# simonmeister/UnFlow

Hardware: AMD Instinct MI355X
Metric: image-pairs/s (fwd+bwd) FlowNetC 384x512 (higher is better)
Workload: dtype f32; 1 GPU; FlowNetC unsupervised step: bidirectional fwd + census/2nd-order loss pyramid + bwd + L2/Adam, 4 pairs/GPU, 384x512, 441-ch correlation (BASELINE configs[1]); global_batch=4, height=384, width=512, parallelism=dp1, hipgraph=True

## Files before the change

unflow_amd/csrc/conv_igemm.hip:

```cpp
#include "igemm_shared.h"
#include "options.h"

namespace {
using namespace igemm;

constexpr int LDK = BK + 4;

struct GatherParams : GatherGeom {
  const float* src;
  const float* w;
  const float* bias;
  float* dst;
  float* partial;
  const float* act_src;
  int lds, ldd, ld_act, act_lo, act_hi;
  int nsplit;
  int leaky, accumulate;
  unsigned cs_magic;
  PlaneOut pl;
};

__device__ __forceinline__ float4 ldg4(const float* p) { return *reinterpret_cast<const float4*>(p); }

typedef __bf16 bf16x8 __attribute__((ext_vector_type(8)));
constexpr bool kEarlyLoads = true;
constexpr int LDH = BK;
__device__ __forceinline__ int swz_off(int row, int kquad) {
  return row * LDH + 8 * ((kquad >> 1) ^ ((row >> 2) & 3)) + 4 * (kquad & 1);
}
__device__ __forceinline__ void split_store(unsigned short* __restrict__ dst, int plane_stride, const float4 v) {
  const unsigned h0 = cvt_pk_bf16(v.x, v.y), h1 = cvt_pk_bf16(v.z, v.w);
  const float r0 = v.x - __uint_as_float(h0 << 16), r1 = v.y - __uint_as_float(h0 & 0xffff0000u);
  const float r2 = v.z - __uint_as_float(h1 << 16), r3 = v.w - __uint_as_float(h1 & 0xffff0000u);
  const unsigned m0 = cvt_pk_bf16(r0, r1), m1 = cvt_pk_bf16(r2, r3);
  const float s0 = r0 - __uint_as_float(m0 << 16), s1 = r1 - __uint_as_float(m0 & 0xffff0000u);
  const float s2 = r2 - __uint_as_float(m1 << 16), s3 = r3 - __uint_as_float(m1 & 0xffff0000u);
  *reinterpret_cast<uint2*>(dst) = make_uint2(h0, h1);
  *reinterpret_cast<uint2*>(dst + plane_stride) = make_uint2(m0, m1);
  *reinterpret_cast<uint2*>(dst + 2 * plane_stride) = make_uint2(cvt_pk_bf16(s0, s1), cvt_pk_bf16(s2, s3));
}

template <int BM, int BN, int WM, int WN, bool B_NK, int MATH = 0>
__global__ __launch_bounds__(256) void igemm_gather_kernel(const GatherParams p) {
  constexpr int TM = WM / 32, TN = WN / 32;
  constexpr int WAVES_N = BN / WN;
  static_assert((BM / WM) * WAVES_N == 4, "4 waves");
  constexpr int A_ELEMS = BM * LDK;
  constexpr int A_PLANE = BM * LDH, B_PLANE = BN * LDH;
  constexpr int AR = BM / 32;
  constexpr int BR_NK = BN / 32;
  constexpr int KG = 256 / BN;
  constexpr int BQ_KN = 8 / KG;
  constexpr int NB = B_NK ? BR_NK : BQ_KN;

  extern __shared__ __attribute__((aligned(16))) float smem[];
  float* As = smem;
  float* Bs = smem + A_ELEMS;
  unsigned short* Ah = reinterpret_cast<unsigned short*>(smem);
  unsigned short* Bh = Ah + 3 * A_PLANE;
  int* pix = MATH ? reinterpret_cast<int*>(Bh + 3 * B_PLANE) : reinterpret_cast<int*>(smem + A_ELEMS + BN * LDK);

  const int tid = threadIdx.x, lane = tid & 63, wid = tid >> 6;
  const int wm = wid / WAVES_N, wn = wid % WAVES_N;
  const int cls_id = blockIdx.z % p.ncls, split = blockIdx.z / p.ncls;
  const TapClass tc = p.cls[cls_id];
  const int M = p.B * p.Hg * p.Wg;
  const int m0 = blockIdx.x * BM, n0 = blockIdx.y * BN;
  const int ntaps = tc.nty * tc.ntx;
  const int Cq = p.Cs >> 2;
  const int Ktot = ntaps * p.Cs;
  const int KT = (Ktot + BK - 1) / BK;
  const int kt_per = (KT + p.nsplit - 1) / p.nsplit;
  const int kt0 = split * kt_per;
  const int kt1 = min(KT, kt0 + kt_per);

  const __amdgpu_buffer_rsrc_t src_rs =
      make_rsrc(p.src, ((size_t)p.B * p.Hs * p.Ws - 1) * (size_t)p.lds * 4 + (size_t)p.Cs * 4);
  const __amdgpu_buffer_rsrc_t w_rs = make_rsrc(p.w, (size_t)p.wtaps * p.Cs * p.N * 4);

  const int kq = tid & 7;
  int a_y[AR], a_x[AR], a_lin[AR];
#pragma unroll
  for (int i = 0; i < AR; i++) {
    const int m = m0 + (tid >> 3) + 32 * i;
    if (m < M) {
      const int xg = m % p.Wg, t = m / p.Wg;
      const int yg = t % p.Hg, b = t / p.Hg;
      a_y[i] = yg * p.sm;
      a_x[i] = xg * p.sm;
      a_lin[i] = b * p.Hs * p.Ws + a_y[i] * p.Ws + a_x[i];
    } else {
      a_y[i] = -(1 << 28);
      a_x[i] = 0;
      a_lin[i] = 0;
    }
  }
  if (tid < BM) {
    const int m = m0 + tid;
    int v = -1;
    if (m < M) {
      const int xg = m % p.Wg, t = m / p.Wg;
      const int yg = t % p.Hg, b = t / p.Hg;
      v = (b * p.Hd + yg * p.so + tc.py) * p.Wd + xg * p.so + tc.px;
    }
    pix[tid] = v;
  }
  int b_row[NB];
  int kn_voff = 0;
  int kn_kg = 0;
  if constexpr (B_NK) {
#pragma unroll
    for (int i = 0; i < NB; i++) {
      const int n = n0 + (tid >> 3) + 32 * i;
      b_row[i] = n < p.N ? n * p.Cs * 4 : OOB_MARK;
    }
  } else {
    const int n = n0 + (tid % BN);
    kn_voff = n < p.N ? n * 4 : OOB_MARK;
    kn_kg = __builtin_amdgcn_readfirstlane(tid / BN);
  }
  const int lds4 = p.lds * 4;

  const int adv_t = 8 / Cq, adv_c = 8 - adv_t * Cq;
  const unsigned ntx_magic = (65536u + (unsigned)tc.ntx - 1u) / (unsigned)tc.ntx;
  int q_tap, q_c4;
  {
    const unsigned q = (unsigned)kt0 * 8u + (unsigned)kq;
    q_tap = (int)(q / (unsigned)Cq);
    q_c4 = (int)(q - (unsigned)q_tap * (unsigned)Cq);
  }
  bool live = kt0 < kt1;

  float4 ra[AR];
  float4 rb[NB];
  int dy, dx, a_tile, w_tile;

  auto piece_begin = [&]() {
    const int ty = (int)(((unsigned)q_tap * ntx_magic) >> 16), tx = q_tap - ty * tc.ntx;
    const bool kvalid = live && q_tap < ntaps;
    dy = tc.dy0 + ty * p.dstep;
    dx = tc.dx0 + tx * p.dstep;
    const int cofs = q_c4 * 16;
    a_tile = kvalid ? (dy * p.Ws + dx) * lds4 + cofs : OOB_MARK;
    if constexpr (B_NK) {
      const int widx = (tc.ky0 + ty * p.kstep) * p.KW + tc.kx0 + tx * p.kstep;
      w_tile = kvalid ? widx * p.N * p.Cs * 4 + cofs : OOB_MARK;
    }
  };
  auto piece_a = [&](int i, float4* RA) {
    const int y = a_y[i] + dy, x = a_x[i] + dx;
    const bool inb = (unsigned)y < (unsigned)p.Hs && (unsigned)x < (unsigned)p.Ws;
    const int voff = inb ? a_lin[i] * lds4 + a_tile : OOB_MARK;
    RA[i] = buf_ld4(src_rs, voff, 0);
  };
  auto piece_b = [&](int i, int kt_next, float4* RB) {
    if constexpr (B_NK) {
      RB[i] = buf_ld4(w_rs, b_row[i] + w_tile, 0);
    } else {
      const int kk = kt_next * BK + 4 * (kn_kg + KG * i);
      float v[4];
#pragma unroll
      for (int j = 0; j < 4; j++) v[j] = buf_ld1(w_rs, kn_voff, min(kk + j, Ktot - 1) * p.N * 4);
      RB[i] = make_float4(v[0], v[1], v[2], v[3]);
    }
  };
  auto piece_end = [&]() {
    q_c4 += adv_c;
    q_tap += adv_t;
    const bool wrap = q_c4 >= Cq;
    q_c4 -= wrap ? Cq : 0;
    q_tap += wrap ? 1 : 0;
  };
  auto piece_set = [&](int step, int kt_next, float4* RA, float4* RB) {
    if (step == 0) piece_begin();
    if (step >= 1 && step <= AR) piece_a(step - 1, RA);
    if (step > AR && step <= AR + NB) piece_b(step - AR - 1, kt_next, RB);
    if (step == AR + NB + 1) piece_end();
  };
  auto piece = [&](int step, int kt_next) { piece_set(step, kt_next, ra, rb); };
  static_assert(AR + NB + 2 <= 16, "pieces must fit the 16 steps");

  auto store_set = [&](const float4* RA, const float4* RB) {
#pragma unroll
    for (int i = 0; i < AR; i++) split_store(Ah + swz_off((tid >> 3) + 32 * i, kq), A_PLANE, RA[i]);
    if constexpr (B_NK) {
#pragma unroll
      for (int i = 0; i < BR_NK; i++) split_store(Bh + swz_off((tid >> 3) + 32 * i, kq), B_PLANE, RB[i]);
    } else {
#pragma unroll
      for (int i = 0; i < BQ_KN; i++) split_store(Bh + swz_off(tid % BN, (tid / BN) + KG * i), B_PLANE, RB[i]);
    }
  };
  auto store_tile = [&]() {
    if constexpr (MATH == 1) {
      store_set(ra, rb);
      return;
    }
#pragma unroll
    for (int i = 0; i < AR; i++)
      *reinterpret_cast<float4*>(As + ((tid >> 3) + 32 * i) * LDK + kq * 4) = ra[i];
    if constexpr (B_NK) {
#pragma unroll
      for (int i = 0; i < BR_NK; i++)
        *reinterpret_cast<float4*>(Bs + ((tid >> 3) + 32 * i) * LDK + kq * 4) = rb[i];
    } else {
#pragma unroll
      for (int i = 0; i < BQ_KN; i++)
        *reinterpret_cast<float4*>(Bs + (tid % BN) * LDK + 4 * ((tid / BN) + KG * i)) = rb[i];
    }
  };

  f32x16 acc[TM][TN];
#pragma unroll
  for (int i = 0; i < TM; i++)
#pragma unroll
    for (int j = 0; j < TN; j++)
#pragma unroll
      for (int r = 0; r < 16; r++) acc[i][j][r] = 0.f;

  const int l31 = lane & 31, lh = lane >> 5;
#pragma unroll
  for (int st = 0; st < 16; st++) piece(st, kt0);
  store_tile();
  __syncthreads();
  const float* a_rd = As + (wm * WM + l31) * LDK + 16 * lh;
  const float* b_rd = Bs + (wn * WN + l31) * LDK + 16 * lh;
  const unsigned short* ah_rd = Ah + (wm * WM + l31) * LDH;
  const unsigned short* bh_rd = Bh + (wn * WN + l31) * LDH;
  const int gsw = lh ^ ((l31 >> 2) & 3);
  constexpr bool EARLY_LOADS = kEarlyLoads;
  auto mfma_phase = [&](int kload, float4* RA, float4* RB) {
#pragma unroll
    for (int slab = 0; slab < 2; slab++) {
      bf16x8 av[3][TM], bv[3][TN];
#pragma unroll
      for (int pl = 0; pl < 3; pl++) {
#pragma unroll
        for (int i = 0; i < TM; i++)
          av[pl][i] = *reinterpret_cast<const bf16x8*>(ah_rd + pl * A_PLANE + i * 32 * LDH + 8 * (gsw ^ (2 * slab)));
#pragma unroll
        for (int j = 0; j < TN; j++)
          bv[pl][j] = *reinterpret_cast<const bf16x8*>(bh_rd + pl * B_PLANE + j * 32 * LDH + 8 * (gsw ^ (2 * slab)));
      }
      constexpr int ta[6] = {2, 0, 1, 1, 0, 0}, tb[6] = {0, 2, 1, 0, 1, 0};
#pragma unroll
      for (int t = 0; t < 6; t++) {
#pragma unroll
        for (int i = 0; i < TM; i++)
#pragma unroll
          for (int j = 0; j < TN; j++)
            acc[i][j] = __builtin_amdgcn_mfma_f32_32x32x16_bf16(av[ta[t]][i], bv[tb[t]][j], acc[i][j], 0, 0, 0);
        if (EARLY_LOADS) {
          piece_set(2 * (slab * 6 + t), kload, RA, RB);
          piece_set(2 * (slab * 6 + t) + 1, kload, RA, RB);
        } else {
          piece_set(slab * 6 + t, kload, RA, RB);
        }
        __builtin_amdgcn_sched_barrier(0);
      }
    }
    if (!EARLY_LOADS) {
#pragma unroll
      for (int st = 12; st < 16; st++) piece_set(st, kload, RA, RB);
    }
  };
  for (int kt = kt0; kt < kt1; kt++) {
    live = kt + 1 < kt1;
    if constexpr (MATH == 1) {
      mfma_phase(kt + 1, ra, rb);
    } else {
#pragma unroll
    for (int j4 = 0; j4 < 4; j4++) {
      float4 av[TM], bv[TN];
#pragma unroll
      for (int i = 0; i < TM; i++) av[i] = *reinterpret_cast<const float4*>(a_rd + i * 32 * LDK + 4 * j4);
#pragma unroll
      for (int j = 0; j < TN; j++) bv[j] = *reinterpret_cast<const float4*>(b_rd + j * 32 * LDK + 4 * j4);
#pragma unroll
      for (int e = 0; e < 4; e++) {
#pragma unroll
        for (int i = 0; i < TM; i++)
#pragma unroll
          for (int j = 0; j < TN; j++)
            acc[i][j] = __builtin_amdgcn_mfma_f32_32x32x2f32((&av[i].x)[e], (&bv[j].x)[e], acc[i][j], 0, 0, 0);
        piece(j4 * 4 + e, kt + 1);
        __builtin_amdgcn_sched_barrier(0);
      }
    }
    }
    __syncthreads();
    store_tile();
    __syncthreads();
  }

  const bool to_partial = p.nsplit > 1;
#pragma unroll
  for (int i = 0; i < TM; i++)
#pragma unroll
    for (int r = 0; r < 16; r++) {
      const int row = wm * WM + i * 32 + (r & 3) + 8 * (r >> 2) + 4 * lh;
      const int px = pix[row];
      if (px < 0) continue;
#pragma unroll
// ... 1248 lines not shown
  }
}


struct GatherPlan {
  int cfg;
  int nsplit;
};

inline bool conv_math_bf16x3() { return !unflow::options().conv_math_fp32; }

inline bool wgrad_math_bf16x3() { return conv_math_bf16x3() && !unflow::options().wgrad_math_fp32; }

inline GatherPlan plan_gather(const GatherParams& p) {
  GatherPlan pl;
  const long M = (long)p.B * p.Hg * p.Wg;
  if (p.N <= 32) pl.cfg = 2;
  else if (p.N <= 64) pl.cfg = 1;
  else pl.cfg = 0;
  int maxtaps = 0;
  for (int c = 0; c < p.ncls; c++) maxtaps = max(maxtaps, p.cls[c].nty * p.cls[c].ntx);
  const int KT = (maxtaps * p.Cs + BK - 1) / BK;
  const int min_kt = max(1, unflow::options().gather_min_kt);
  const int max_by_k = min(16, KT / min_kt > 0 ? KT / min_kt : 1);
  if (pl.cfg == 0) {
    const long b128 = ((M + 127) / 128) * ((p.N + 127) / 128) * p.ncls;
    if (b128 * max_by_k < 384) pl.cfg = 2;
  }
  const int bm = pl.cfg == 2 ? 64 : 128, bn = pl.cfg == 0 ? 128 : 64;
  const int slots = 256 * (pl.cfg == 0 ? 3 : pl.cfg == 1 ? 4 : 6);
  const long blocks = ((M + bm - 1) / bm) * ((p.N + bn - 1) / bn) * p.ncls;
  pl.nsplit = fill_one_round(blocks, slots, max_by_k);
  return pl;
}

inline size_t gather_partial_bytes(const GatherParams& p, int nsplit) {
  return nsplit > 1 ? (size_t)nsplit * p.B * p.Hd * p.Wd * p.N * sizeof(float) : 0;
}

inline int wgrad_cfg(const WgradParams& p) { return p.Cb <= 64 ? 1 : 0; }

inline int plan_wgrad(const WgradParams& p) {
  const int Mp = p.KH * p.KW * p.Ca;
  const int cfg = wgrad_cfg(p);
  const int bn = cfg == 1 ? 64 : 128;
  const long blocks = (long)cdiv(Mp, 128) * cdiv(p.Cb, bn);
  const long S = (long)p.B * p.Hg * p.Wg;
  const int KT = (int)((S + BK - 1) / BK);
  const int min_kt = max(1, unflow::options().wgrad_min_kt);
  const int max_by_k = min(256, KT / min_kt > 0 ? KT / min_kt : 1);
  const bool b3 = wgrad_math_bf16x3();
  const int slots = 256 * (b3 ? (cfg == 1 ? 4 : 3) : cfg == 1 ? 5 : 4);
  return fill_one_round(blocks, slots, max_by_k);
}

inline size_t wgrad_partial_bytes(const WgradParams& p, int nsplit) {
  const size_t n = (size_t)p.KH * p.KW * p.Ca * p.Cb;
  return nsplit > 1 ? (size_t)nsplit * n * sizeof(float) + reduce_scratch_bytes(n, nsplit) : 0;
}

inline int skinny_wgrad_chunks(long npix, int Cin) {
  const long colblocks = (Cin / 4 + 63) / 64;
  long c = (4096 + colblocks - 1) / colblocks;
  c = min(c, max((long)1, npix / 8));
  return (int)min(c, (long)1024);
}

inline int head_strip(int B, int H, int W, int k, int Cout) {
  if (k != 3 || Cout != 2) return 0;
  if (W % 8 == 0 && (long)B * H * W >= 16384) return 8;
  return W % 4 == 0 ? 4 : 0;
}
inline int head_wgrad_blocks(int B, int H, int W, int Cin, int S, int* strips_per_wave) {
  const long nstrips = (long)B * H * (W / S);
  const long colblocks = (Cin / 4 + 63) / 64;
  long blocks = min((long)1024, max((long)1, 1024 / colblocks));
  long spw = max((long)(nstrips >= 4096 ? 4 : 1), (nstrips + blocks * 4 - 1) / (blocks * 4));
  blocks = (nstrips + spw * 4 - 1) / (spw * 4);
  *strips_per_wave = (int)spw;
  return (int)blocks;
}

constexpr size_t COLSUM_SCRATCH_BYTES(int C) { return (size_t)REDUCE_FAN * C * sizeof(float) + 512; }

template <int BM, int BN, int WM, int WN, bool B_NK, int MATH = 0>
int launch_gather_cfg(const GatherParams& p, hipStream_t st) {
  const int M = p.B * p.Hg * p.Wg;
  const size_t smem = (MATH ? (size_t)3 * (BM + BN) * LDH * sizeof(unsigned short) : (size_t)(BM + BN) * LDK * sizeof(float)) +
                      BM * sizeof(int);
  static DynLdsBook attr_book{};
  (void)ensure_dyn_lds(reinterpret_cast<const void*>(&igemm_gather_kernel<BM, BN, WM, WN, B_NK, MATH>), (int)smem, attr_book);
  dim3 grid(cdiv(M, BM), cdiv(p.N, BN), p.ncls * p.nsplit);
  igemm_gather_kernel<BM, BN, WM, WN, B_NK, MATH><<<grid, 256, smem, st>>>(p);
  return launch_status();
}

template <bool B_NK>
int run_gather(GatherParams& p, void* ws, size_t ws_bytes, hipStream_t st) {
  p.cs_magic = magic_u32((unsigned)p.Cs);
  const GatherPlan pl = plan_gather(p);
  p.nsplit = pl.nsplit;
  p.partial = nullptr;
  if (p.nsplit > 1) {
    if (!ws || ws_bytes < gather_partial_bytes(p, p.nsplit)) p.nsplit = 1;
    else p.partial = reinterpret_cast<float*>(ws);
  }
  int code;
  switch (pl.cfg) {
    case 0: code = conv_math_bf16x3() ? launch_gather_cfg<128, 128, 64, 64, B_NK, 1>(p, st)
                                      : launch_gather_cfg<128, 128, 64, 64, B_NK>(p, st); break;
    case 1: code = conv_math_bf16x3() ? launch_gather_cfg<128, 64, 64, 32, B_NK, 1>(p, st)
                                      : launch_gather_cfg<128, 64, 64, 32, B_NK>(p, st); break;
    default: code = launch_gather_cfg<64, 64, 32, 32, B_NK>(p, st); break;
  }
  if (code != UNFLOW_OK) return code;
  if (p.nsplit > 1) {
    const size_t total = (size_t)p.B * p.Hd * p.Wd * p.N;
    const uintptr_t al = reinterpret_cast<uintptr_t>(p.dst) | reinterpret_cast<uintptr_t>(p.partial) |
                         reinterpret_cast<uintptr_t>(p.act_src);
    const bool vec = p.N % 4 == 0 && p.ldd % 4 == 0 && (!p.act_src || p.ld_act % 4 == 0) && (al & 15) == 0;
    if (vec) splitk_reduce_epilogue_kernel<<<stream_grid((long)(total / 4)), 256, 0, st>>>(p);
    else splitk_reduce_epilogue_scalar_kernel<<<stream_grid((long)total), 256, 0, st>>>(p);
    return launch_status();
  }
  return UNFLOW_OK;
}

template <int BM, int BN, int WM, int WN>
int launch_wgrad_b3_cfg(const WgradParams& p, hipStream_t st) {
  const int Mp = p.KH * p.KW * p.Ca;
  const size_t smem = (size_t)3 * (BM + BN) * LDH * sizeof(unsigned short);
  static DynLdsBook attr_book{};
  (void)ensure_dyn_lds(reinterpret_cast<const void*>(&igemm_wgrad_b3_kernel<BM, BN, WM, WN>), (int)smem, attr_book);
  dim3 grid(cdiv(Mp, BM), cdiv(p.Cb, BN), p.nsplit);
  igemm_wgrad_b3_kernel<BM, BN, WM, WN><<<grid, 256, smem, st>>>(p);
  return launch_status();
}

template <int BM, int BN, int WM, int WN>
int launch_wgrad_cfg(const WgradParams& p, hipStream_t st) {
  const int Mp = p.KH * p.KW * p.Ca;
  const size_t smem = (size_t)(BK * BM + BK * BN) * sizeof(float);
  static DynLdsBook attr_book{};
  (void)ensure_dyn_lds(reinterpret_cast<const void*>(&igemm_wgrad_kernel<BM, BN, WM, WN>), (int)smem, attr_book);
  dim3 grid(cdiv(Mp, BM), cdiv(p.Cb, BN), p.nsplit);
  igemm_wgrad_kernel<BM, BN, WM, WN><<<grid, 256, smem, st>>>(p);
  return launch_status();
}

int run_wgrad(WgradParams& p, void* ws, size_t ws_bytes, size_t* used, hipStream_t st) {
  p.ca_magic = magic_u32((unsigned)p.Ca);
  const size_t wsize = (size_t)p.KH * p.KW * p.Ca * p.Cb;
  int ns = plan_wgrad(p);
  if (ns > 1 && (!ws || ws_bytes < wgrad_partial_bytes(p, ns))) {
    ns = ws ? (int)min((size_t)REDUCE_FAN, ws_bytes / (wsize * sizeof(float))) : 1;
    if (ns < 1) ns = 1;
  }
  p.nsplit = ns;
  p.partial = ns > 1 ? reinterpret_cast<float*>(ws) : nullptr;
  *used = wgrad_partial_bytes(p, ns);
  const int cfg = wgrad_cfg(p);
  const bool b3 = wgrad_math_bf16x3();
  const int code = b3 ? (cfg == 1 ? launch_wgrad_b3_cfg<128, 64, 64, 32>(p, st) : launch_wgrad_b3_cfg<128, 128, 64, 64>(p, st))
                 : cfg == 1 ? launch_wgrad_cfg<128, 64, 64, 32>(p, st)
                            : launch_wgrad_cfg<128, 128, 64, 64>(p, st);
  if (code != UNFLOW_OK) return code;
  if (ns > 1) return reduce_partials(p.partial, p.partial + (size_t)ns * wsize, p.out, wsize, ns, st);
  return UNFLOW_OK;
}

int run_colsum(const float* dz, int ld, long npix, int C, float* out, void* ws, size_t ws_bytes, size_t ws_used,
               hipStream_t st) {
  int chunks = (int)min((long)REDUCE_FAN, max((long)1, npix / 256));
  float* part = nullptr;
  const size_t need = (size_t)chunks * C * sizeof(float);
  const size_t off = (ws_used + 255) & ~(size_t)255;
  if (ws && ws_bytes >= off + need) part = reinterpret_cast<float*>(reinterpret_cast<char*>(ws) + off);
  else chunks = 1;
  dim3 grid(cdiv(C, 64), chunks);
  colsum_partial_kernel<<<grid, 256, 0, st>>>(dz, ld, npix, C, chunks == 1 ? out : part);
  if (chunks > 1) sum_partials_kernel<<<stream_grid(C), 256, 0, st>>>(part, out, (size_t)C, chunks, REDUCE_FAN);
  return launch_status();
}

}

int unflow_conv2d_fwd_po(const float* x, int ldx, const float* w, const float* bias, float* y, int ldy, int B, int H, int W,
                         int Cin, int Cout, int k, int stride, int leaky, const igemm::PlaneOut& po, void* workspace,
                         size_t workspace_bytes, unflow_stream_t stream);
int unflow_conv2d_bwd_data_po(const float* dz, int lddz, const float* w, float* dx, int lddx, int B, int H, int W, int Cin,
                              int Cout, int k, int stride, int accumulate, const float* act_src, int ld_act, int act_lo,
                              int act_hi, const igemm::PlaneOut& po, void* workspace, size_t workspace_bytes,
                              unflow_stream_t stream);
int unflow_conv2d_transpose_fwd_po(const float* x, int ldx, const float* w, const float* bias, float* y, int ldy, int B, int H,
                                   int W, int Cin, int Cout, int leaky, const igemm::PlaneOut& po, void* workspace,
                                   size_t workspace_bytes, unflow_stream_t stream);
int unflow_conv2d_transpose_bwd_data_po(const float* dz, int lddz, const float* w, float* dx, int lddx, int B, int H, int W,
                                        int Cin, int Cout, int accumulate, const float* act_src, int ld_act, int act_lo,
                                        int act_hi, const igemm::PlaneOut& po, void* workspace, size_t workspace_bytes,
                                        unflow_stream_t stream);

UNFLOW_API size_t unflow_conv_workspace_bytes(int B, int H, int W, int Cin, int Cout, int k, int stride) {
  if (B <= 0 || H <= 0 || W <= 0 || Cin <= 0 || Cout <= 0 || k <= 0 || stride <= 0) return 0;
  size_t need = 4096;
  const int cmax = max(Cin, Cout);
  if (Cout <= 4 || Cin < 4) {
    const size_t wsz = (size_t)k * k * max(Cin, 4) * max(Cout, 2);
    const int ch = skinny_wgrad_chunks((long)B * H * W, max(Cin, 4));
    need = max(need, (size_t)ch * wsz * sizeof(float) + reduce_scratch_bytes(wsz, ch));
  } else {
    GatherParams g{};
    build_conv_fwd(g, B, H, W, Cin, Cout, k, stride);
    need = max(need, gather_partial_bytes(g, plan_gather(g).nsplit));
    GatherParams d{};
    if ((stride == 1 || stride == 2) && build_conv_dgrad(d, B, H, W, Cin, Cout, k, stride) == UNFLOW_OK)
      need = max(need, gather_partial_bytes(d, plan_gather(d).nsplit));
    WgradParams w{};
    build_conv_wgrad(w, B, H, W, Cin, Cout, k, stride);
    need = max(need, wgrad_partial_bytes(w, plan_wgrad(w)));
    if (k == 4 && stride == 2 && H % 2 == 0 && W % 2 == 0) {
      GatherParams tf{};
      build_deconv_fwd(tf, B, H / 2, W / 2, Cin, Cout);
      need = max(need, gather_partial_bytes(tf, plan_gather(tf).nsplit));
      GatherParams td{};
      build_deconv_dgrad(td, B, H / 2, W / 2, Cin, Cout);
      need = max(need, gather_partial_bytes(td, plan_gather(td).nsplit));
      WgradParams tw{};
      build_deconv_wgrad(tw, B, H / 2, W / 2, Cin, Cout);
      need = max(need, wgrad_partial_bytes(tw, plan_wgrad(tw)));
    }
  }
  return need + COLSUM_SCRATCH_BYTES(cmax) + 1024;
}

UNFLOW_API int unflow_conv2d_fwd(const float* x, int ldx, const float* w, const float* bias, float* y, int ldy, int B,
                                 int H, int W, int Cin, int Cout, int k, int stride, int leaky, void* workspace,
                                 size_t workspace_bytes, unflow_stream_t stream) {
  return unflow_conv2d_fwd_po(x, ldx, w, bias, y, ldy, B, H, W, Cin, Cout, k, stride, leaky, igemm::PlaneOut{}, workspace,
                              workspace_bytes, stream);
}

int unflow_conv2d_fwd_po(const float* x, int ldx, const float* w, const float* bias, float* y, int ldy, int B, int H, int W,
                         int Cin, int Cout, int k, int stride, int leaky, const igemm::PlaneOut& po, void* workspace,
                         size_t workspace_bytes, unflow_stream_t stream) {
  if (!x || !w || !y) return UNFLOW_ERR_NULL;
  if (B <= 0 || H <= 0 || W <= 0 || Cin <= 0 || Cout <= 0 || k <= 0 || stride <= 0) return UNFLOW_ERR_SHAPE;
  if (Cin % 4 != 0 || ldx % 4 != 0 || ldx < Cin || ldy < Cout) return UNFLOW_ERR_UNSUPPORTED;
  hipStream_t st = as_stream(stream);
  if (Cout <= 4) {
    if (stride != 1 || leaky) return UNFLOW_ERR_UNSUPPORTED;
    int pt, pl, Ho, Wo;
    same_pads(H, k, 1, &pt, &Ho);
    same_pads(W, k, 1, &pl, &Wo);
    SkinnyParams p{x, ldx, w, bias, y, ldy, B, H, W, Cin, k, pt, pl};
    const int S = head_strip(B, H, W, k, Cout);
    if (S == 8) {
      const long jobs = (long)B * cdiv(H, HT_R) * (W / 8);
      head3_fwd_tile_kernel<<<(int)((jobs + 3) / 4), 256, 0, st>>>(p);
      return launch_status();
    }
    if (S == 4) {
      head3_fwd_strip_kernel<4, true><<<B * H * (W / 4), 256, 0, st>>>(p);
      return launch_status();
    }
    const long waves = (long)B * H * W;
    const int grid = (int)min((long)4096, (waves + 3) / 4);
    if (Cout == 2) skinny_conv_fwd_kernel<2><<<grid, 256, 0, st>>>(p);
    else if (Cout == 1) skinny_conv_fwd_kernel<1><<<grid, 256, 0, st>>>(p);
    else if (Cout == 4) skinny_conv_fwd_kernel<4><<<grid, 256, 0, st>>>(p);
    else return UNFLOW_ERR_UNSUPPORTED;
    return launch_status();
  }
  if (Cout % 4 != 0) return UNFLOW_ERR_UNSUPPORTED;
  GatherParams p{};
  build_conv_fwd(p, B, H, W, Cin, Cout, k, stride);
  p.src = x; p.w = w; p.bias = bias; p.dst = y; p.act_src = nullptr;
  p.lds = ldx; p.ldd = ldy; p.leaky = leaky; p.accumulate = 0;
  p.pl = po;
  return run_gather<false>(p, workspace, workspace_bytes, st);
}

UNFLOW_API int unflow_conv2d_bwd_data(const float* dz, int lddz, const float* w, float* dx, int lddx, int B, int H,
                                      int W, int Cin, int Cout, int k, int stride, int accumulate,
                                      const float* act_src, int ld_act, int act_lo, int act_hi, void* workspace,
                                      size_t workspace_bytes, unflow_stream_t stream) {
  return unflow_conv2d_bwd_data_po(dz, lddz, w, dx, lddx, B, H, W, Cin, Cout, k, stride, accumulate, act_src, ld_act, act_lo,
                                   act_hi, igemm::PlaneOut{}, workspace, workspace_bytes, stream);
}

int unflow_conv2d_bwd_data_po(const float* dz, int lddz, const float* w, float* dx, int lddx, int B, int H, int W, int Cin,
                              int Cout, int k, int stride, int accumulate, const float* act_src, int ld_act, int act_lo,
                              int act_hi, const igemm::PlaneOut& po, void* workspace, size_t workspace_bytes,
                              unflow_stream_t stream) {
  if (!dz || !w || !dx) return UNFLOW_ERR_NULL;
  if (B <= 0 || H <= 0 || W <= 0 || Cin <= 0 || Cout <= 0 || k <= 0 || (stride != 1 && stride != 2)) return UNFLOW_ERR_SHAPE;
  if (Cin % 4 != 0 || lddx < Cin || lddz < Cout) return UNFLOW_ERR_UNSUPPORTED;
  hipStream_t st = as_stream(stream);
  if (Cout <= 4) {
    if (stride != 1) return UNFLOW_ERR_UNSUPPORTED;
    int pt, pl, Ho, Wo;
    same_pads(H, k, 1, &pt, &Ho);
    same_pads(W, k, 1, &pl, &Wo);
    SkinnyBwdParams p{dz, lddz, w, dx, lddx, act_src, ld_act, act_lo, act_hi, accumulate, B, H, W, Cin, k, pt, pl, po};
    const int S = (lddx % 4 == 0 && (!act_src || ld_act % 4 == 0)) ? head_strip(B, H, W, k, Cout) : 0;
    if (S) {
      const int strips = W / S, ns = 1;
      const long jobs = (long)B * H * (strips / ns) * cdiv(Cin / 4, 64);
      if (S == 8) head3_dgrad_strip_kernel<8><<<(int)((jobs + 3) / 4), 256, 0, st>>>(p, ns);
      else head3_dgrad_strip_kernel<4><<<(int)((jobs + 3) / 4), 256, 0, st>>>(p, ns);
      return launch_status();
    }
    const long total = (long)B * H * W * (Cin / 4);
    if (Cout == 2) skinny_conv_dgrad_kernel<2><<<stream_grid(total), 256, 0, st>>>(p);
    else if (Cout == 1) skinny_conv_dgrad_kernel<1><<<stream_grid(total), 256, 0, st>>>(p);
    else if (Cout == 4) skinny_conv_dgrad_kernel<4><<<stream_grid(total), 256, 0, st>>>(p);
    else return UNFLOW_ERR_UNSUPPORTED;
    return launch_status();
  }
  if (Cout % 4 != 0 || lddz % 4 != 0) return UNFLOW_ERR_UNSUPPORTED;
  if (k == 1 && stride == 1 && Cout == PW_CO && lddx % 4 == 0 && (!act_src || ld_act % 4 == 0) &&
      (reinterpret_cast<uintptr_t>(dx) & 15) == 0 && (reinterpret_cast<uintptr_t>(act_src) & 15) == 0 &&
      (reinterpret_cast<uintptr_t>(w) & 15) == 0) {
    SkinnyBwdParams sp{dz, lddz, w, dx, lddx, act_src, ld_act, act_lo, act_hi, accumulate, B, H, W, Cin, 1, 0, 0, po};
    const long jobs = (((long)B * H * W + PW_S - 1) / PW_S) * cdiv(Cin / 4, 64);
    pointwise32_dgrad_kernel<<<(int)((jobs + 3) / 4), 256, 0, st>>>(sp);
    return launch_status();
  }
  GatherParams p{};
  const int bc = build_conv_dgrad(p, B, H, W, Cin, Cout, k, stride);
  if (bc != UNFLOW_OK) return bc;
  p.src = dz; p.w = w; p.bias = nullptr; p.dst = dx; p.act_src = act_src;
  p.lds = lddz; p.ldd = lddx; p.ld_act = ld_act; p.act_lo = act_lo; p.act_hi = act_hi;
  p.leaky = 0; p.accumulate = accumulate;
  p.pl = po;
  return run_gather<true>(p, workspace, workspace_bytes, st);
}

UNFLOW_API int unflow_conv2d_bwd_filter(const float* x, int ldx, const float* dz, int lddz, float* dw, float* dbias,
                                        int B, int H, int W, int Cin, int Cout, int k, int stride, void* workspace,
                                        size_t workspace_bytes, unflow_stream_t stream) {
  if (!x || !dz || !dw) return UNFLOW_ERR_NULL;
  if (B <= 0 || H <= 0 || W <= 0 || Cin <= 0 || Cout <= 0 || k <= 0 || stride <= 0) return UNFLOW_ERR_SHAPE;
  if (Cin % 4 != 0 || ldx % 4 != 0 || ldx < Cin || lddz < Cout) return UNFLOW_ERR_UNSUPPORTED;
  int pt, pl, Ho, Wo;
  same_pads(H, k, stride, &pt, &Ho);
  same_pads(W, k, stride, &pl, &Wo);
  hipStream_t st = as_stream(stream);
  size_t used = 0;
  if (Cout <= 4) {
    if (stride != 1 || k != 3 || Cout != 2) return UNFLOW_ERR_UNSUPPORTED;
    const long npix = (long)B * H * W;
    const size_t wsz = (size_t)9 * Cin * Cout;
    const int S = head_strip(B, H, W, k, Cout);
    const bool strip = S != 0;
    int spw = 1;
    const int chunks = strip ? head_wgrad_blocks(B, H, W, Cin, S, &spw) : skinny_wgrad_chunks(npix, Cin);
    used = (size_t)chunks * wsz * sizeof(float) + reduce_scratch_bytes(wsz, chunks);
    if (!workspace || workspace_bytes < used) return UNFLOW_ERR_WORKSPACE;
    SkinnyWgradParams p{x, ldx, dz, lddz, reinterpret_cast<float*>(workspace), B, H, W, Cin, pt, pl};
    dim3 grid(cdiv(Cin / 4, 64), chunks);
    if (S == 8) head3_wgrad_strip_kernel<8><<<grid, 256, 0, st>>>(p, spw);
    else if (S == 4) head3_wgrad_strip_kernel<4><<<grid, 256, 0, st>>>(p, spw);
    else skinny_conv_wgrad3_kernel<2><<<grid, 64, 0, st>>>(p);
    const int rc = reduce_partials(p.partial, p.partial + (size_t)chunks * wsz, dw, wsz, chunks, st);
    if (rc != UNFLOW_OK) return rc;
  } else {
    if (Cout % 4 != 0 || lddz % 4 != 0) return UNFLOW_ERR_UNSUPPORTED;
    WgradParams p{};
    build_conv_wgrad(p, B, H, W, Cin, Cout, k, stride);
    p.src = x; p.dst = dz; p.out = dw; p.lds = ldx; p.ldd = lddz;
    const int code = run_wgrad(p, workspace, workspace_bytes, &used, st);
    if (code != UNFLOW_OK) return code;
  }
  if (dbias) return run_colsum(dz, lddz, (long)B * Ho * Wo, Cout, dbias, workspace, workspace_bytes, used, st);
  return launch_status();
}

UNFLOW_API int unflow_conv2d_transpose_fwd(const float* x, int ldx, const float* w, const float* bias, float* y,
                                           int ldy, int B, int H, int W, int Cin, int Cout, int leaky, void* workspace,
                                           size_t workspace_bytes, unflow_stream_t stream) {
  return unflow_conv2d_transpose_fwd_po(x, ldx, w, bias, y, ldy, B, H, W, Cin, Cout, leaky, igemm::PlaneOut{}, workspace,
                                        workspace_bytes, stream);
}

int unflow_conv2d_transpose_fwd_po(const float* x, int ldx, const float* w, const float* bias, float* y, int ldy, int B, int H,
                                   int W, int Cin, int Cout, int leaky, const igemm::PlaneOut& po, void* workspace,
                                   size_t workspace_bytes, unflow_stream_t stream) {
  if (!x || !w || !y) return UNFLOW_ERR_NULL;
  if (B <= 0 || H <= 0 || W <= 0 || Cin <= 0 || Cout <= 0) return UNFLOW_ERR_SHAPE;
  hipStream_t st = as_stream(stream);
  if (Cin == 2 && Cout == 2) {
    if (leaky) return UNFLOW_ERR_UNSUPPORTED;
    tiny_deconv_fwd_kernel<2, 2><<<stream_grid((long)B * 4 * H * W), 256, 0, st>>>(x, ldx, w, bias, y, ldy, B, H, W, po);
    return launch_status();
  }
  if (Cin % 4 != 0 || ldx % 4 != 0 || ldx < Cin || ldy < Cout) return UNFLOW_ERR_UNSUPPORTED;
  GatherParams p{};
  build_deconv_fwd(p, B, H, W, Cin, Cout);
  p.src = x; p.w = w; p.bias = bias; p.dst = y; p.act_src = nullptr;
  p.lds = ldx; p.ldd = ldy; p.leaky = leaky; p.accumulate = 0;
  p.pl = po;
  return run_gather<true>(p, workspace, workspace_bytes, st);
}

UNFLOW_API int unflow_conv2d_transpose_bwd_data(const float* dz, int lddz, const float* w, float* dx, int lddx, int B,
                                                int H, int W, int Cin, int Cout, int accumulate, const float* act_src,
                                                int ld_act, int act_lo, int act_hi, void* workspace,
                                                size_t workspace_bytes, unflow_stream_t stream) {
  return unflow_conv2d_transpose_bwd_data_po(dz, lddz, w, dx, lddx, B, H, W, Cin, Cout, accumulate, act_src, ld_act, act_lo,
                                             act_hi, igemm::PlaneOut{}, workspace, workspace_bytes, stream);
}

int unflow_conv2d_transpose_bwd_data_po(const float* dz, int lddz, const float* w, float* dx, int lddx, int B, int H, int W,
                                        int Cin, int Cout, int accumulate, const float* act_src, int ld_act, int act_lo,
                                        int act_hi, const igemm::PlaneOut& po, void* workspace, size_t workspace_bytes,
                                        unflow_stream_t stream) {
  if (!dz || !w || !dx) return UNFLOW_ERR_NULL;
  if (B <= 0 || H <= 0 || W <= 0 || Cin <= 0 || Cout <= 0) return UNFLOW_ERR_SHAPE;
  hipStream_t st = as_stream(stream);
  if (Cin == 2 && Cout == 2) {
    if (act_src) return UNFLOW_ERR_UNSUPPORTED;
    tiny_deconv_dgrad_kernel<2, 2><<<stream_grid((long)B * H * W), 256, 0, st>>>(dz, lddz, w, dx, lddx, accumulate, B, H, W);
    return launch_status();
  }
  if (Cout % 4 != 0 || Cin % 4 != 0 || lddz % 4 != 0 || lddz < Cout || lddx < Cin) return UNFLOW_ERR_UNSUPPORTED;
  GatherParams p{};
  build_deconv_dgrad(p, B, H, W, Cin, Cout);
  p.src = dz; p.w = w; p.bias = nullptr; p.dst = dx; p.act_src = act_src;
  p.lds = lddz; p.ldd = lddx; p.ld_act = ld_act; p.act_lo = act_lo; p.act_hi = act_hi;
  p.leaky = 0; p.accumulate = accumulate;
  p.pl = po;
  return run_gather<false>(p, workspace, workspace_bytes, st);
}

UNFLOW_API int unflow_conv2d_transpose_bwd_filter(const float* x, int ldx, const float* dz, int lddz, float* dw,
                                                  float* dbias, int B, int H, int W, int Cin, int Cout, void* workspace,
                                                  size_t workspace_bytes, unflow_stream_t stream) {
  if (!x || !dz || !dw) return UNFLOW_ERR_NULL;
  if (B <= 0 || H <= 0 || W <= 0 || Cin <= 0 || Cout <= 0) return UNFLOW_ERR_SHAPE;
  hipStream_t st = as_stream(stream);
  size_t used = 0;
  if (Cin == 2 && Cout == 2) {
    const int blocks = (int)min((long)32, ((long)B * H * W + 255) / 256);
    if (!workspace || workspace_bytes < (size_t)blocks * 64 * sizeof(float)) return UNFLOW_ERR_WORKSPACE;
    float* part = reinterpret_cast<float*>(workspace);
    tiny_deconv_wgrad_kernel<2, 2><<<blocks, 256, 0, st>>>(x, ldx, dz, lddz, part, B, H, W);
    sum_partials_kernel<<<1, 64, 0, st>>>(part, dw, 64, blocks, 128);
    used = (size_t)blocks * 64 * sizeof(float);
  } else {
    if (Cout % 4 != 0 || Cin % 4 != 0 || lddz % 4 != 0 || ldx % 4 != 0) return UNFLOW_ERR_UNSUPPORTED;
    WgradParams p{};
    build_deconv_wgrad(p, B, H, W, Cin, Cout);
    p.src = dz; p.dst = x; p.out = dw; p.lds = lddz; p.ldd = ldx;
    const int code = run_wgrad(p, workspace, workspace_bytes, &used, st);
    if (code != UNFLOW_OK) return code;
  }
  if (dbias) return run_colsum(dz, lddz, (long)B * 4 * H * W, Cout, dbias, workspace, workspace_bytes, used, st);
  return launch_status();
}

static bool flow_wgrad_plan(FlowWgradDesc& d, int kind_in, int B, int H, int W, int Cin) {
  if (kind_in == 1) {
    d.kind = 2; d.colblocks = 1; d.spw = 0; d.wsz = 64;
    d.chunks = (int)min((long)32, ((long)B * H * W + 255) / 256);
    return true;
  }
  const int S = head_strip(B, H, W, 3, 2);
  if (S != 8 && S != 4) return false;
  d.kind = S == 8 ? 0 : 1;
  d.colblocks = cdiv(Cin / 4, 64);
  d.wsz = 9 * Cin * 2;
  const long nstrips = (long)B * H * (W / S);
  const long blocks = min((long)256, max((long)1, nstrips / 16));
  const long spw = (nstrips + blocks * 4 - 1) / (blocks * 4);
  d.spw = (int)spw;
  d.chunks = (int)((nstrips + spw * 4 - 1) / (spw * 4));
  return true;
}

UNFLOW_API size_t unflow_flow_wgrad_batched_workspace_bytes(int n, const int* kind, const int* B, const int* H, const int* W,
                                                            const int* Cin) {
  size_t need = 0;
  for (int i = 0; i < n; i++) {
    FlowWgradDesc d{};
    if (!flow_wgrad_plan(d, kind[i], B[i], H[i], W[i], Cin[i])) return 0;
    need += ((size_t)d.chunks * d.wsz * sizeof(float) + 255) & ~(size_t)255;
  }
  return need;
}

UNFLOW_API int unflow_flow_wgrad_batched(int n, const int* kind, const float* const* x, const int* ldx, const float* const* dz,
                                         const int* lddz, float* const* dw, const int* B, const int* H, const int* W, const int* Cin,
                                         void* workspace, size_t workspace_bytes, unflow_stream_t stream) {
  if (!kind || !x || !ldx || !dz || !lddz || !dw || !B || !H || !W || !Cin) return UNFLOW_ERR_NULL;
  if (n <= 0) return UNFLOW_OK;
  if (n > MAX_FLOW_WGRAD) return UNFLOW_ERR_UNSUPPORTED;
  FlowWgradBatch b{};
  b.n = n;
  size_t off = 0;
  int blocks = 0, rblocks = 0;
  for (int i = 0; i < n; i++) {
    FlowWgradDesc& d = b.d[i];
    if (!x[i] || !dz[i] || !dw[i]) return UNFLOW_ERR_NULL;
    if (B[i] <= 0 || H[i] <= 0 || W[i] <= 0 || Cin[i] <= 0) return UNFLOW_ERR_SHAPE;
    if (kind[i] == 0 && (Cin[i] % 4 != 0 || ldx[i] % 4 != 0 || ldx[i] < Cin[i] || lddz[i] < 2)) return UNFLOW_ERR_UNSUPPORTED;
    if (kind[i] == 1 && Cin[i] != 2) return UNFLOW_ERR_UNSUPPORTED;
    if (!flow_wgrad_plan(d, kind[i], B[i], H[i], W[i], Cin[i])) return UNFLOW_ERR_UNSUPPORTED;
    int pt, pl, ho, wo;
    same_pads(H[i], 3, 1, &pt, &ho);
    same_pads(W[i], 3, 1, &pl, &wo);
    const size_t bytes = ((size_t)d.chunks * d.wsz * sizeof(float) + 255) & ~(size_t)255;
    if (!workspace || off + bytes > workspace_bytes) return UNFLOW_ERR_WORKSPACE;
    d.p = SkinnyWgradParams{x[i], ldx[i], dz[i], lddz[i], reinterpret_cast<float*>(reinterpret_cast<char*>(workspace) + off),
                            B[i], H[i], W[i], Cin[i], pt, pl};
    off += bytes;
    d.out = dw[i];
    d.block0 = blocks;
    blocks += d.chunks * d.colblocks;
    d.rblock0 = rblocks;
    rblocks += cdiv(d.wsz, 16);
  }
  hipStream_t st = as_stream(stream);
  flow_wgrad_batched_kernel<<<blocks, 256, 0, st>>>(b);
  flow_wgrad_sum_kernel<<<rblocks, 256, 0, st>>>(b);
  return launch_status();
}

UNFLOW_API int unflow_leaky_bwd_inplace(float* dy, int lddy, const float* y, int ldy, long npix, int C,
                                        unflow_stream_t stream) {
  if (!dy || !y) return UNFLOW_ERR_NULL;
  if (npix <= 0 || C <= 0) return UNFLOW_OK;
  leaky_bwd_inplace_kernel<<<stream_grid(npix * C), 256, 0, as_stream(stream)>>>(dy, lddy, y, ldy, npix, C);
  return launch_status();
}

UNFLOW_API size_t unflow_colsum_batched_workspace_bytes(int n, const int* C) {
  size_t t = 0;
  for (int i = 0; i < n; i++) t += (size_t)COLSUM_MAX_CHUNKS * C[i];
  return t * sizeof(float) + 256;
}

UNFLOW_API int unflow_colsum_batched(int n, const float* const* x, const int* ld, const long* npix, const int* C,
                                     float* const* out, void* workspace, size_t workspace_bytes,
                                     unflow_stream_t stream) {
  if (!x || !ld || !npix || !C || !out || !workspace) return UNFLOW_ERR_NULL;
  if (n <= 0) return UNFLOW_OK;
  if (n > MAX_COLSUM) return UNFLOW_ERR_UNSUPPORTED;
  if (workspace_bytes < unflow_colsum_batched_workspace_bytes(n, C)) return UNFLOW_ERR_WORKSPACE;
  ColsumBatch d{};
  d.n = n;
  int blocks = 0;
  long poff = 0;
  for (int i = 0; i < n; i++) {
    if (!x[i] || !out[i] || C[i] <= 0 || npix[i] <= 0 || ld[i] < C[i]) return UNFLOW_ERR_SHAPE;
    d.x[i] = x[i]; d.out[i] = out[i]; d.npix[i] = npix[i]; d.ld[i] = ld[i]; d.C[i] = C[i];
    d.chunks[i] = (int)min((long)COLSUM_MAX_CHUNKS, max((long)1, npix[i] / 512));
    d.block0[i] = blocks;
    blocks += ((C[i] + 63) / 64) * d.chunks[i];
    d.part0[i] = poff;
    poff += (long)d.chunks[i] * C[i];
  }
  d.block0[n] = blocks;
  hipStream_t st = as_stream(stream);
  float* part = reinterpret_cast<float*>(workspace);
  colsum_batched_kernel<<<blocks, 256, 0, st>>>(d, part);
  int maxc = 0;
  for (int i = 0; i < n; i++) maxc = max(maxc, C[i]);
  colsum_batched_final_kernel<<<dim3((maxc + 63) / 64, n), 256, 0, st>>>(d, part);
  return launch_status();
}
```

unflow_amd/csrc/options.h:

```cpp
#pragma once

#define UNFLOW_OPTION_LIST(X)                                                                                              \
  X(conv_math_fp32, 0)           \
  X(wgrad_math_fp32, 0)                             \
  X(corr_math_fp32, 0)                                                               \
  X(gather_min_kt, 8)                          \
  X(gather_max_split, 16)                                                           \
  X(wgrad_min_kt, 8)                     \
  X(gather_pp, 1)          \
  X(gather_pp_fill, 60)    \
  X(f16_k64, 1)            \
  X(f16_wgrad_dma, 1)      \
  X(f16_tall, 0)           \
  X(f16_db, 0)             \
  X(gather_tile2d, 1)                                                     \
  X(conv1_direct, 1)       \
  X(halo, 1)                                     \
  X(streamk, 1)                \
  X(streamk_groups, 8)             \
  X(halo_max_split, 16)                                         \
  X(halo_s2, 1)                       \
  X(xcd_swizzle, 1)                                                                        \
  X(wgrad_dma, 1)                                                \
  X(wgrad_pp, 1)                                                     \
  X(corr_nb, 1)                                                               \
  X(corr_rs, 2)            \
  X(corr_wb, 1)                                                                 \
  X(corr_rw, 1)                                                       \
  X(corr_bwd_b128, 1)                                                 \
  X(corr_bwd_rot, -1)              \
  X(corr_bwd_planes, 1)                                                 \
  X(corr_bwd_share, 1)

namespace unflow {
struct Options {
#define X(name, def) int name = def;
  UNFLOW_OPTION_LIST(X)
#undef X
};
Options& options();
}
```

Measured before the change: 659.2 image-pairs/s.

## Route flow-head and pointwise conv dgrad through fp32 MFMA kernel

Adds a new backward-data kernel for the skinny flow-prediction heads (3x3, Cout 1-2) and the 1x1 Cout=32 pointwise convs. It computes them with 32x32x2 fp32 MFMA instructions instead of the scalar strip and pointwise kernels. Each wave forms a 32-pixel by 32-channel tile, transposes the result through LDS, and fuses the accumulate, leaky-ReLU gradient and plane-output stores. It is on by default through a new option. Most MFMA lanes are wasted for Cout 1-2 and the 3x3 loads of dz are scalar gathers, so the gain over the existing tuned kernels is uncertain.

```diff
diff --git a/unflow_amd/csrc/conv_heads_mfma.h b/unflow_amd/csrc/conv_heads_mfma.h
--- /dev/null
+++ b/unflow_amd/csrc/conv_heads_mfma.h
@@ -0,0 +1,19 @@
+#pragma once
+#include "igemm_shared.h"
+
+namespace heads_mfma {
+
+struct DgradArgs {
+  const float* dz; int lddz;
+  const float* w;
+  float* dx; int lddx;
+  const float* act_src; int ld_act, act_lo, act_hi;
+  int accumulate;
+  int B, H, W, Cin, Cout, k;
+  igemm::PlaneOut po;
+};
+
+bool dgrad_eligible(const DgradArgs& a);
+int dgrad(const DgradArgs& a, hipStream_t st);
+
+}
diff --git a/unflow_amd/csrc/conv_heads_mfma.hip b/unflow_amd/csrc/conv_heads_mfma.hip
--- /dev/null
+++ b/unflow_amd/csrc/conv_heads_mfma.hip
@@ -0,0 +1,166 @@
+#include "conv_heads_mfma.h"
+#include "options.h"
+
+namespace {
+using namespace igemm;
+using heads_mfma::DgradArgs;
+
+constexpr int NB = 1;
+constexpr int TP = 32 * NB + 4;
+constexpr int QW = 8 * NB;
+constexpr int SPI = 64 / QW;
+constexpr int NI = 32 / SPI;
+
+__device__ __forceinline__ float4 ldg4(const float* p) { return *reinterpret_cast<const float4*>(p); }
+
+template <int K2>
+__global__ __launch_bounds__(256) void heads_mfma_dgrad_kernel(const DgradArgs p, int ngroups, int ntiles) {
+  __shared__ float turn[4][32 * TP];
+  const int lane = threadIdx.x & 63, n = lane & 31, h = lane >> 5;
+  const long job = (long)__builtin_amdgcn_readfirstlane((int)((blockIdx.x * (long)blockDim.x + threadIdx.x) >> 6));
+  if (job >= (long)ntiles * ngroups) return;
+  const int g = (int)(job % ngroups);
+  const long tile = job / ngroups;
+  const long npix = (long)p.B * p.H * p.W;
+  const long pxl = tile * 32 + n;
+  const bool site_ok = pxl < npix;
+  const long px = site_ok ? pxl : npix - 1;
+
+  float bz[K2];
+  if constexpr (K2 == 9) {
+    const Pix pp = decode_pix((unsigned)px, (unsigned)p.W, (unsigned)p.H);
+    const int co = h < p.Cout ? h : 0;
+#pragma unroll
+    for (int ky = 0; ky < 3; ky++)
+#pragma unroll
+      for (int kx = 0; kx < 3; kx++) {
+        const int oy = pp.y + 1 - ky, ox = pp.x + 1 - kx;
+        const bool ok = site_ok && h < p.Cout && (unsigned)oy < (unsigned)p.H && (unsigned)ox < (unsigned)p.W;
+        const long q = ok ? px + (long)(1 - ky) * p.W + (1 - kx) : px;
+        const float v = p.dz[q * p.lddz + co];
+        bz[ky * 3 + kx] = ok ? v : 0.f;
+      }
+  } else {
+    const float* zp = p.dz + px * p.lddz + 16 * h;
+#pragma unroll
+    for (int q = 0; q < 4; q++) {
+      const float4 t = ldg4(zp + 4 * q);
+      bz[4 * q] = site_ok ? t.x : 0.f; bz[4 * q + 1] = site_ok ? t.y : 0.f;
+      bz[4 * q + 2] = site_ok ? t.z : 0.f; bz[4 * q + 3] = site_ok ? t.w : 0.f;
+    }
+  }
+
+  float wa[NB][K2];
+#pragma unroll
+  for (int bi = 0; bi < NB; bi++) {
+    const int ch = (g * NB + bi) * 32 + n;
+    const bool cok = ch < p.Cin;
+    const int cc = cok ? ch : 0;
+    if constexpr (K2 == 9) {
+      const bool ok = cok && h < p.Cout;
+      const int co = h < p.Cout ? h : 0;
+#pragma unroll
+      for (int t = 0; t < 9; t++) {
+        const float v = p.w[((size_t)t * p.Cin + cc) * p.Cout + co];
+        wa[bi][t] = ok ? v : 0.f;
+      }
+    } else {
+      const float* wp = p.w + (size_t)cc * 32 + 16 * h;
+#pragma unroll
+      for (int q = 0; q < 4; q++) {
+        const float4 t = ldg4(wp + 4 * q);
+        wa[bi][4 * q] = cok ? t.x : 0.f; wa[bi][4 * q + 1] = cok ? t.y : 0.f;
+        wa[bi][4 * q + 2] = cok ? t.z : 0.f; wa[bi][4 * q + 3] = cok ? t.w : 0.f;
+      }
+    }
+  }
+
+  const int cq = g * (32 * NB) + 4 * (lane % QW);
+  const bool c_ok = cq < p.Cin;
+  const bool a_any = p.act_src && c_ok && cq + 3 >= p.act_lo && cq < p.act_hi;
+  const bool ax = cq >= p.act_lo && cq < p.act_hi, ay = cq + 1 >= p.act_lo && cq + 1 < p.act_hi;
+  const bool az = cq + 2 >= p.act_lo && cq + 2 < p.act_hi, aw = cq + 3 >= p.act_lo && cq + 3 < p.act_hi;
+  const long s0 = tile * 32 + lane / QW;
+  float4 old[NI], act[NI];
+#pragma unroll
+  for (int i = 0; i < NI; i++) {
+    const long s = s0 + SPI * i;
+    const bool ok = c_ok && s < npix;
+    old[i] = make_float4(0.f, 0.f, 0.f, 0.f);
+    act[i] = make_float4(1.f, 1.f, 1.f, 1.f);
+    if (p.accumulate && ok) old[i] = ldg4(p.dx + s * p.lddx + cq);
+    if (a_any && s < npix) {
+      const float4 t = ldg4(p.act_src + s * p.ld_act + cq);
+      if (ax) act[i].x = t.x;
+      if (ay) act[i].y = t.y;
+      if (az) act[i].z = t.z;
+      if (aw) act[i].w = t.w;
+    }
+  }
+
+  f32x16 acc[NB];
+#pragma unroll
+  for (int bi = 0; bi < NB; bi++) {
+#pragma unroll
+    for (int i = 0; i < 16; i++) acc[bi][i] = 0.f;
+    if ((g * NB + bi) * 32 < p.Cin) {
+#pragma unroll
+      for (int t = 0; t < K2; t++) acc[bi] = __builtin_amdgcn_mfma_f32_32x32x2f32(wa[bi][t], bz[t], acc[bi], 0, 0, 0);
+    }
+  }
+
+  float* tl = turn[threadIdx.x >> 6];
+#pragma unroll
+  for (int bi = 0; bi < NB; bi++)
+#pragma unroll
+    for (int j = 0; j < 4; j++)
+      *reinterpret_cast<float4*>(tl + n * TP + 32 * bi + 8 * j + 4 * h) =
+          make_float4(acc[bi][4 * j], acc[bi][4 * j + 1], acc[bi][4 * j + 2], acc[bi][4 * j + 3]);
+  __builtin_amdgcn_wave_barrier();
+
+#pragma unroll
+  for (int i = 0; i < NI; i++) {
+    const long s = s0 + SPI * i;
+    float4 v = *reinterpret_cast<const float4*>(tl + (lane / QW + SPI * i) * TP + 4 * (lane % QW));
+    if (p.accumulate) { v.x += old[i].x; v.y += old[i].y; v.z += old[i].z; v.w += old[i].w; }
+    if (p.act_src) {
+      v.x *= leaky_grad_from_out(act[i].x); v.y *= leaky_grad_from_out(act[i].y);
+      v.z *= leaky_grad_from_out(act[i].z); v.w *= leaky_grad_from_out(act[i].w);
+    }
+    if (c_ok && s < npix) {
+      *reinterpret_cast<float4*>(p.dx + s * p.lddx + cq) = v;
+      store_planes4(p.po, (size_t)s, cq, v);
+    }
+  }
+}
+
+inline bool al16(const void* q) { return (reinterpret_cast<uintptr_t>(q) & 15) == 0; }
+
+}
+
+namespace heads_mfma {
+
+bool dgrad_eligible(const DgradArgs& a) {
+  const bool head = a.k == 3 && (a.Cout == 1 || a.Cout == 2);
+  const bool pw = a.k == 1 && a.Cout == 32;
+  if (!head && !pw) return false;
+  if (a.Cin % 4 != 0 || a.lddx % 4 != 0 || !al16(a.dx)) return false;
+  if (a.act_src && (a.ld_act % 4 != 0 || !al16(a.act_src))) return false;
+  if (pw && (a.lddz % 4 != 0 || !al16(a.dz) || !al16(a.w))) return false;
+  const long npix = (long)a.B * a.H * a.W;
+  if (npix > 0x7fffff00L) return false;
+  return ((npix + 31) / 32) * cdiv(a.Cin, 32 * NB) <= 0x7fffff00L;
+}
+
+int dgrad(const DgradArgs& a, hipStream_t st) {
+  const long npix = (long)a.B * a.H * a.W;
+  const int ntiles = (int)((npix + 31) / 32);
+  const int ngroups = cdiv(a.Cin, 32 * NB);
+  const long jobs = (long)ntiles * ngroups;
+  const int grid = (int)((jobs + 3) / 4);
+  if (a.k == 3) heads_mfma_dgrad_kernel<9><<<grid, 256, 0, st>>>(a, ngroups, ntiles);
+  else heads_mfma_dgrad_kernel<16><<<grid, 256, 0, st>>>(a, ngroups, ntiles);
+  return launch_status();
+}
+
+}
diff --git a/unflow_amd/csrc/conv_igemm.hip b/unflow_amd/csrc/conv_igemm.hip
--- a/unflow_amd/csrc/conv_igemm.hip
+++ b/unflow_amd/csrc/conv_igemm.hip
@@ -1,4 +1,5 @@
 #include "igemm_shared.h"
+#include "conv_heads_mfma.h"
 #include "options.h"
 
 namespace {
@@ -1853,6 +1854,10 @@
     same_pads(H, k, 1, &pt, &Ho);
     same_pads(W, k, 1, &pl, &Wo);
     SkinnyBwdParams p{dz, lddz, w, dx, lddx, act_src, ld_act, act_lo, act_hi, accumulate, B, H, W, Cin, k, pt, pl, po};
+    if (unflow::options().head_mfma) {
+      const heads_mfma::DgradArgs ha{dz, lddz, w, dx, lddx, act_src, ld_act, act_lo, act_hi, accumulate, B, H, W, Cin, Cout, k, po};
+      if (heads_mfma::dgrad_eligible(ha)) return heads_mfma::dgrad(ha, st);
+    }
     const int S = (lddx % 4 == 0 && (!act_src || ld_act % 4 == 0)) ? head_strip(B, H, W, k, Cout) : 0;
     if (S) {
       const int strips = W / S, ns = 1;
@@ -1872,6 +1877,10 @@
   if (k == 1 && stride == 1 && Cout == PW_CO && lddx % 4 == 0 && (!act_src || ld_act % 4 == 0) &&
       (reinterpret_cast<uintptr_t>(dx) & 15) == 0 && (reinterpret_cast<uintptr_t>(act_src) & 15) == 0 &&
       (reinterpret_cast<uintptr_t>(w) & 15) == 0) {
+    if (unflow::options().head_mfma) {
+      const heads_mfma::DgradArgs ha{dz, lddz, w, dx, lddx, act_src, ld_act, act_lo, act_hi, accumulate, B, H, W, Cin, Cout, 1, po};
+      if (heads_mfma::dgrad_eligible(ha)) return heads_mfma::dgrad(ha, st);
+    }
     SkinnyBwdParams sp{dz, lddz, w, dx, lddx, act_src, ld_act, act_lo, act_hi, accumulate, B, H, W, Cin, 1, 0, 0, po};
     const long jobs = (((long)B * H * W + PW_S - 1) / PW_S) * cdiv(Cin / 4, 64);
     pointwise32_dgrad_kernel<<<(int)((jobs + 3) / 4), 256, 0, st>>>(sp);
diff --git a/unflow_amd/csrc/options.h b/unflow_amd/csrc/options.h
--- a/unflow_amd/csrc/options.h
+++ b/unflow_amd/csrc/options.h
@@ -30,7 +30,8 @@
   X(corr_bwd_b128, 1)                                                 \
   X(corr_bwd_rot, -1)              \
   X(corr_bwd_planes, 1)                                                 \
-  X(corr_bwd_share, 1)
+  X(corr_bwd_share, 1)                    \
+  X(head_mfma, 1)
 
 namespace unflow {
 struct Options {
```

After: 661.9 image-pairs/s (median of 6 runs). No clear change (+0.4%).
